# sglang-npu/DeepGEMM_Ascend

Hardware: AMD Instinct MI355X
Metric: fp8 TFLOPS + % MFMA peak, 4096^3 block-scaled GEMM; grouped-GEMM tok/s at 1/2/4/8 GPU (higher is better)
Workload: dtype bf16

## Files before the change

### deepgemm_ascend_amd/csrc/dga_launch_menu_l.hip

```cpp
#include <cstdlib>
#include "dga_fp8_menu_impl.hpp"
#include "gemm_fp8_bf16x_grouped_kernel.hpp"
namespace dga {

template <bool KTAIL, bool BNT, bool STAG, bool IDX = false>
static int launch_bf16x_grouped_one(const GemmParams &p, hipStream_t stream)
{
    typedef GemmCfg<128, 256, 2, 4, 3> Cfg;
    constexpr int kLds = Cfg::LDS_BYTES + (IDX ? 256 * 16 : 0);
    const int64_t tiles = static_cast<int64_t>(p.groups) * p.tiles_m * p.tiles_n;
    const unsigned grid = static_cast<unsigned>(std::min<int64_t>(tiles, device_cus()));
    return launch_kernel<gemm_fp8_bf16x_grouped_kernel<KTAIL, BNT, STAG, IDX>>(grid, Cfg::NT, kLds, stream, p);
}

int launch_bf16x_grouped(const GemmParams &p, hipStream_t stream)
{
    if (p.tail_sub || p.m_indices || p.launch_tiles > 0 || p.splitk > 1 || p.kb_n < 2) return DGA_E_TILING;
    const bool nt = p.b_nt != 0;
#ifdef DGA_BXG_KNOBS
    if (const char *e = std::getenv("DGA_BXG_KNOB"); e && (std::atoi(e) & 2)) {
        if (p.k % 128) return nt ? launch_bf16x_grouped_one<true, true, false>(p, stream) : launch_bf16x_grouped_one<true, false, false>(p, stream);
        return nt ? launch_bf16x_grouped_one<false, true, false>(p, stream) : launch_bf16x_grouped_one<false, false, false>(p, stream);
    }
#endif
    if (p.row_index) {
        if (p.k % 128) return nt ? launch_bf16x_grouped_one<true, true, true, true>(p, stream) : launch_bf16x_grouped_one<true, false, true, true>(p, stream);
        return nt ? launch_bf16x_grouped_one<false, true, true, true>(p, stream) : launch_bf16x_grouped_one<false, false, true, true>(p, stream);
    }
    if (p.k % 128) return nt ? launch_bf16x_grouped_one<true, true, true>(p, stream) : launch_bf16x_grouped_one<true, false, true>(p, stream);
    return nt ? launch_bf16x_grouped_one<false, true, true>(p, stream) : launch_bf16x_grouped_one<false, false, true>(p, stream);
}
}
```

### deepgemm_ascend_amd/csrc/gemm_fp8_bf16x_grouped_kernel.hpp

```cpp
#pragma once
#include "gemm_fp8_kernel.hpp"

namespace dga {

template <bool KTAIL, bool BNT, bool STAGGER = true, bool INDEXED = false>
__global__ void __launch_bounds__(512) __attribute__((amdgpu_waves_per_eu(2, 2)))
gemm_fp8_bf16x_grouped_kernel(const GemmParams p)
{
    typedef GemmCfg<128, 256, 2, 4, 3> Cfg;
    constexpr int BM = Cfg::kBM, BN = Cfg::kBN, WN = Cfg::kWN, TM = Cfg::TM, TN = Cfg::TN, DNT = Cfg::DNT;
    constexpr int NL = Cfg::LOADS_PER_STAGE, LAGT = 2, RING = 4, NT = Cfg::NT;
    static_assert(Cfg::NT == 512 && DNT == 512 && TM == 4 && TN == 4 && Cfg::SC_ITERS == 1 && Cfg::STAGES == 3, "the grouped schedule");
    typedef __bf16 v8bf __attribute__((ext_vector_type(8)));
    extern __shared__ __attribute__((aligned(16))) uint8_t smem[];

    const int tid = threadIdx.x, lane = tid & 63;
    const int wave = __builtin_amdgcn_readfirstlane(tid >> 6);
    const int wm = wave / WN, wn = wave % WN;
    const int li = lane & 15, kg = lane >> 4;
    const int KB = p.kb_n;

    const int tiles_per_group = p.tiles_m * p.tiles_n;
    const int total = p.groups * tiles_per_group;
    int first = 0, count = total, step = gridDim.x, slot = blockIdx.x;
    if (p.xcd_remap) {
        const int xcd = blockIdx.x & 7, q = total >> 3, r = total & 7;
        first = xcd < r ? xcd * (q + 1) : r * (q + 1) + (xcd - r) * q;
        count = q + (xcd < r ? 1 : 0);
        step = ((int)gridDim.x - xcd + 7) >> 3;
        slot = blockIdx.x >> 3;
    }
    struct Tile { int g, M, m0, n0; };
    typedef const __attribute__((address_space(4))) int32_t *const_i32_ptr;
    const const_i32_ptr masked_m_c = (const_i32_ptr)p.masked_m;
    auto seek = [&](int &local, Tile &t) -> bool {
        for (; local < count; local += step) {
            const int tile = first + local;
            const int g = tile / tiles_per_group;
            const int t_in = tile - g * tiles_per_group;
            const int gm = p.raster_group;
            const int per = gm * p.tiles_n;
            const int band = t_in / per;
            const int row0 = band * gm;
            const int rows = min(p.tiles_m - row0, gm);
            const int loc = t_in - band * per;
            const int tm = row0 + loc % rows, tn = loc / rows;
            const int M = p.masked_m ? min(masked_m_c[g], p.m) : p.m;
            const int m0 = tm * BM;
            if (m0 >= M) continue;
            t.g = g; t.M = M; t.m0 = m0; t.n0 = tn * BN;
            return true;
        }
        return false;
    };

    const uint32_t lds0 = (uint32_t)(uintptr_t)(lptr_t)smem;
    constexpr uint32_t kOutOfRange = 0x80000000u;
    const int a_col = ((tid & 7) ^ swz_a(tid >> 3)) * 16;
    const int b_col = ((tid & 7) ^ swz_b(tid >> 3)) * 16;
    v4i a_rsrc, b_rsrc;
    uint32_t a_voff[Cfg::A_ITERS], b_voff[Cfg::B_ITERS];
    const float *sc_src;
    int kbf = 0;
    bool fill_valid = true;
    constexpr bool indexed = INDEXED;
    static_assert(Cfg::A_ITERS == 2, "partner slot: two A offsets and the scale pointer");
    uint32_t *const pslot = reinterpret_cast<uint32_t *>(smem + Cfg::LDS_BYTES) + (tid & (DNT / 2 - 1)) * 4;
    auto a_off_of = [&](const Tile &t, int it, int td) -> uint32_t {
        const int row = (it * DNT + td) >> 3;
        if (row >= t.M - t.m0) return kOutOfRange;
        const uint32_t r = indexed ? (uint32_t)p.row_index[(int64_t)t.g * p.m + t.m0 + row] : (uint32_t)row;
        return r * (uint32_t)p.lda + a_col;
    };
    auto b_off_of = [&](const Tile &t, int it, int td) -> uint32_t {
        const int row = (it * DNT + td) >> 3;
        return (uint32_t)min(row, p.n - 1 - t.n0) * (uint32_t)p.ldb + b_col;
    };
    auto sc_of = [&](const Tile &t, int td) -> const float * {
        const float *SFA = p.sfa + (int64_t)t.g * p.sfa_gs, *SFB = p.sfb + (int64_t)t.g * p.sfb_gs;
        if (td >= BM) return SFB + (int64_t)min(t.n0 / 128 + min(td - BM, 7), p.nb_n - 1) * p.kb_n;
        const int mr = min(t.m0 + td, t.M - 1);
        return SFA + (indexed ? p.row_index[(int64_t)t.g * p.m + mr] : (int64_t)mr) * p.sfa_ld;
    };
    Tile T{}, F{};
    auto set_fill = [&](const Tile &t) {
        a_rsrc = indexed ? make_rsrc(p.a, p.a_bytes)
                         : make_rsrc(p.a + (int64_t)t.g * p.a_gs + (int64_t)t.m0 * p.lda, (int64_t)(t.M - t.m0) * p.lda);
        b_rsrc = make_rsrc(p.b + (int64_t)t.g * p.b_gs + (int64_t)t.n0 * p.ldb, (int64_t)(p.n - t.n0) * p.ldb);
#pragma unroll
        for (int it = 0; it < Cfg::A_ITERS; ++it) a_voff[it] = a_off_of(t, it, tid);
#pragma unroll
        for (int it = 0; it < Cfg::B_ITERS; ++it) b_voff[it] = b_off_of(t, it, tid);
        sc_src = sc_of(t, tid);
        if constexpr (INDEXED) {
            if (wm == 1) {
                const uint64_t ps = (uint64_t)(uintptr_t)sc_of(t, tid - DNT / 2);
                *reinterpret_cast<v4i *>(pslot) = v4i{(int)a_off_of(t, 0, tid - DNT / 2), (int)a_off_of(t, 1, tid - DNT / 2), (int)(uint32_t)ps, (int)(uint32_t)(ps >> 32)};
            }
        }
    };
    auto refill = [&](int idx, int stage, auto sc) {
        constexpr int S = decltype(sc)::value;
        const int w = wave - 4 * S, td = tid - S * (DNT / 2);
        const uint32_t sa = lds0 + stage * Cfg::STAGE_BYTES + w * 1024;
        const int k0 = kbf * 128;
        if (idx < Cfg::A_ITERS) {
            uint32_t voff = fill_valid ? (S ? (INDEXED ? pslot[idx] : a_off_of(F, idx, td)) : a_voff[idx]) : kOutOfRange;
            if constexpr (KTAIL) voff = (k0 + a_col < p.k) ? voff : kOutOfRange;
            dma16(voff, a_rsrc, (uint32_t)k0, sa + idx * DNT * 16);
        } else if (idx < Cfg::A_ITERS + Cfg::B_ITERS) {
            const int it = idx - Cfg::A_ITERS;
            uint32_t voff = fill_valid ? (S ? b_off_of(F, it, td) : b_voff[it]) : kOutOfRange;
            if constexpr (KTAIL) voff = (k0 + b_col < p.k) ? voff : kOutOfRange;
            if constexpr (BNT) dma16_nt(voff, b_rsrc, (uint32_t)k0, sa + Cfg::A_BYTES + it * DNT * 16);
            else dma16(voff, b_rsrc, (uint32_t)k0, sa + Cfg::A_BYTES + it * DNT * 16);
        } else {
            const float *src = S ? (INDEXED ? reinterpret_cast<const float *>((uintptr_t)*reinterpret_cast<const uint64_t *>(pslot + 2)) : sc_of(F, td)) : sc_src;
            dma4(src + (fill_valid ? kbf : KB - 1), lds0 + stage * Cfg::STAGE_BYTES + Cfg::A_BYTES + Cfg::B_BYTES + w * 256);
        }
    };
    constexpr std::integral_constant<int, 0> kOwn{};
    constexpr std::integral_constant<int, 1> kPartner{};

    const int a_row = wm * (BM / Cfg::kWM) + li;
    const int a_off0 = a_row * 128 + ((kg ^ swz_a(a_row)) * 16);
    const int a_off1 = a_row * 128 + (((kg + 4) ^ swz_a(a_row)) * 16);
    const int b_row = wn * (BN / WN) + 8 * (li >> 2) + (li & 3);
    const int b_off0 = Cfg::A_BYTES + b_row * 128 + ((kg ^ swz_b(b_row)) * 16);
    const int b_off1 = Cfg::A_BYTES + b_row * 128 + (((kg + 4) ^ swz_b(b_row)) * 16);
    const int sa_off = Cfg::A_BYTES + Cfg::B_BYTES + (wm * (BM / Cfg::kWM) + li) * 4;
    const int sb_off = Cfg::A_BYTES + Cfg::B_BYTES + (BM + (wn * (BN / WN)) / 128) * 4;

    v4f acc[TM][TN];
    v4f part[RING];
    v4i afx[TM][4], bfx[2][4];
    v4i braw[2], araw[2][2];
    float s_cur[TM], s_old[TM];

    auto wait_all_but = [&](auto base, int extra) {
        constexpr int B = decltype(base)::value;
        if (extra >= 8) wait_vmcnt<B + 8>();
        else if (extra >= 6) wait_vmcnt<B + 6>();
        else if (extra >= 4) wait_vmcnt<B + 4>();
        else if (extra >= 2) wait_vmcnt<B + 2>();
        else wait_vmcnt<B>();
    };
    auto wait_landed = [&](int younger, int extra) {
        if (younger >= 2 * NL) wait_all_but(std::integral_constant<int, 2 * NL>{}, extra);
        else if (younger >= NL) wait_all_but(std::integral_constant<int, NL>{}, extra);
        else wait_all_but(std::integral_constant<int, 0>{}, extra);
    };

    int local = slot;
    if (!seek(local, T)) return;
    F = T;
    set_fill(F);
#pragma unroll
    for (int d = 0; d < 2; ++d) {
#pragma unroll
        for (int idx = 0; idx < NL; ++idx) refill(idx, d, kOwn);
        ++kbf;
    }
    int cur = 0;
    DGA_STAMP_DECL
    DGA_STAMP_CLOCK(6, 7);
    DGA_STAMP_START();
    int stores_pending = 0;
    int younger = NL;

    auto advance_fill = [&]() {
        if (kbf == KB) {
            local += step;
            fill_valid = seek(local, F);
            if (fill_valid) set_fill(F);
            kbf = 0;
        }
    };

    auto run_tile = [&](auto Lc, auto lonec, auto stagc) __attribute__((always_inline)) {
        constexpr int L = decltype(Lc)::value;
        constexpr bool lone = decltype(lonec)::value;
        constexpr bool STAG = decltype(stagc)::value;
        constexpr int G = 4 * (L > 0 ? L : 1);
        constexpr int TILES = (L > 0 ? L : 1) * TN;
        constexpr int SP = L > 0 ? L : 1;
        constexpr int HALF = 2 * TILES;
        static_assert(1 + (NL - 1) * SP < HALF, "the refill fits half a block");
        static_assert(!(STAG && (lone || L == 0)), "a staggered wave multiplies and issues its own pieces");
        if constexpr (L > 0) {
#pragma unroll
            for (int i = 0; i < L; ++i)
#pragma unroll
                for (int j = 0; j < TN; ++j) acc[i][j] = v4f{0.f, 0.f, 0.f, 0.f};
#pragma unroll
            for (int i = 0; i < RING; ++i) part[i] = v4f{0.f, 0.f, 0.f, 0.f};
#pragma unroll
            for (int i = 0; i < L; ++i) s_old[i] = 0.f;
        }
        auto head = [&](const uint8_t *sc) __attribute__((always_inline)) {
            araw[0][0] = *(const v4i *)(sc + a_off0);
            araw[0][1] = *(const v4i *)(sc + a_off1);
            braw[0] = *(const v4i *)(sc + b_off0);
            braw[1] = *(const v4i *)(sc + b_off1);
            if constexpr (L > 1) {
                araw[1][0] = *(const v4i *)(sc + a_off0 + 2048);
                araw[1][1] = *(const v4i *)(sc + a_off1 + 2048);
            }
            const float sfb0 = *(const float *)(sc + sb_off);
            float sa[L > 0 ? L : 1];
#pragma unroll
            for (int i = 0; i < L; ++i) sa[i] = *(const float *)(sc + sa_off + i * 64);
            __builtin_amdgcn_sched_barrier(0);
#pragma unroll
            for (int c = 0; c < 8; ++c) bx_convert(braw, bfx[0], c);
            braw[0] = *(const v4i *)(sc + b_off0 + b_frag_off(1));
#pragma unroll
            for (int c = 8; c < 16; ++c) bx_convert(braw, bfx[0], c);
            braw[1] = *(const v4i *)(sc + b_off1 + b_frag_off(1));
#pragma unroll
            for (int c = 0; c < 16; ++c) bx_convert(araw[0], afx[0], c);
            if constexpr (L > 2) {
                araw[0][0] = *(const v4i *)(sc + a_off0 + 2 * 2048);
                araw[0][1] = *(const v4i *)(sc + a_off1 + 2 * 2048);
            }
#pragma unroll
            for (int i = 0; i < L; ++i) s_cur[i] = sa[i] * sfb0;
            __builtin_amdgcn_sched_barrier(0);
        };
        auto gaps = [&](auto u0c, auto u1c, auto refillc, const uint8_t *sc, int fill) __attribute__((always_inline)) {
            constexpr int U0 = decltype(u0c)::value, U1 = decltype(u1c)::value;
            constexpr bool REFILL = decltype(refillc)::value;
#pragma unroll
            for (int u = U0; u < U1; ++u) {
                const int t = u >> 2, q = u & 3, nt = t / L, mt = t % L, g = u % G;
                part[t % RING] = __builtin_amdgcn_mfma_f32_16x16x32_bf16(
                    __builtin_bit_cast(v8bf, bfx[nt & 1][q]), __builtin_bit_cast(v8bf, afx[mt][q]),
                    q == 0 ? v4f{0.f, 0.f, 0.f, 0.f} : part[t % RING], 0, 0, 0);
                __builtin_amdgcn_sched_barrier(0);
                if (REFILL && u - U0 >= 1 && (u - U0 - 1) % SP == 0 && (u - U0 - 1) / SP < NL) refill((u - U0 - 1) / SP, fill, kOwn);
                if (nt == 0 && mt + 1 < L) {
#pragma unroll
                    for (int c = 0; c < 4; ++c) bx_convert(araw[(mt + 1) & 1], afx[mt + 1], 4 * q + c);
                    if (q == 3 && mt + 3 < L) {
                        araw[(mt + 1) & 1][0] = *(const v4i *)(sc + a_off0 + (mt + 3) * 2048);
                        araw[(mt + 1) & 1][1] = *(const v4i *)(sc + a_off1 + (mt + 3) * 2048);
                    }
                }
                if (nt + 1 < TN) {
#pragma unroll
                    for (int c = 16 * g / G; c < 16 * (g + 1) / G; ++c) bx_convert(braw, bfx[(nt + 1) & 1], c);
                    if (nt + 2 < TN) {
                        if (g == G / 2 - 1) braw[0] = *(const v4i *)(sc + b_off0 + b_frag_off(nt + 2));
                        if (g == G - 1) braw[1] = *(const v4i *)(sc + b_off1 + b_frag_off(nt + 2));
                    }
                }
                {
                    const int j = t >= LAGT ? t - LAGT : TILES + t - LAGT, jn = j / L, jm = j % L;
                    const float sv = t >= LAGT ? s_cur[jm] : s_old[jm];
                    acc[jm][jn][q] = __builtin_fmaf(part[j % RING][q], sv, acc[jm][jn][q]);
                }
                __builtin_amdgcn_sched_barrier(0);
            }
        };
        constexpr std::integral_constant<int, 0> kU0{};
        constexpr std::integral_constant<int, HALF> kUh{};
        constexpr std::integral_constant<int, 4 * TILES> kU1{};
        auto end_of_block = [&]() {
#pragma unroll
            for (int i = 0; i < L; ++i) s_old[i] = s_cur[i];
        };
        auto top = [&](int kb) __attribute__((always_inline)) -> int {
            DGA_STAMP(0);
            wait_landed(younger, kb < 2 ? stores_pending : 0);
            DGA_STAMP(1);
            __builtin_amdgcn_s_barrier();
            asm volatile("" ::: "memory");
            DGA_STAMP(2);
            advance_fill();
            return cur >= 1 ? cur - 1 : 2;
        };
        auto next_block = [&]() {
            ++kbf;
            cur = cur == 2 ? 0 : cur + 1;
        };
        if constexpr (STAG) {
            {
                const int fill = top(0);
                younger = NL;
#pragma unroll
                for (int idx = 0; idx < NL; ++idx) refill(idx, fill, kOwn);
                const uint8_t *sc = smem + cur * Cfg::STAGE_BYTES;
                head(sc);
                gaps(kU0, kUh, std::false_type{}, sc, fill);
                next_block();
            }
            for (int kb = 1; kb < KB; ++kb) {
                const int fill = top(kb);
                const uint8_t *sc = smem + cur * Cfg::STAGE_BYTES;
                gaps(kUh, kU1, std::true_type{}, sc, fill);
                end_of_block();
                head(sc);
                DGA_STAMP(3);
                gaps(kU0, kUh, std::false_type{}, sc, fill);
                DGA_STAMP(4);
                next_block();
            }
            gaps(kUh, kU1, std::false_type{}, smem, 0);
            end_of_block();
        } else {
            for (int kb = 0; kb < KB; ++kb) {
                const int fill = top(kb);
                if constexpr (L == 0) {
#pragma unroll
                    for (int idx = 0; idx < NL; ++idx) {
                        if (lone) refill(idx, fill, kPartner);
                        refill(idx, fill, kOwn);
                    }
                    younger = lone ? 2 * NL : NL;
                } else {
                    younger = lone ? 0 : NL;
                    const uint8_t *sc = smem + cur * Cfg::STAGE_BYTES;
                    head(sc);
                    DGA_STAMP(3);
                    if constexpr (lone) gaps(kU0, kU1, std::false_type{}, sc, fill);
                    else gaps(kU0, kU1, std::true_type{}, sc, fill);
                    end_of_block();
                    DGA_STAMP(4);
                }
                next_block();
            }
        }
        stores_pending = 0;
        if constexpr (L > 0) {
#pragma unroll
            for (int t = 0; t < LAGT; ++t) {
                const int j = TILES + t - LAGT, jn = j / L, jm = j % L;
#pragma unroll
                for (int q = 0; q < 4; ++q) acc[jm][jn][q] = __builtin_fmaf(part[j % RING][q], s_old[jm], acc[jm][jn][q]);
            }
            uint16_t *C = p.out + (int64_t)T.g * p.c_gs;
            const int m_row = T.m0 + wm * (BM / Cfg::kWM) + li;
            const int n_base = T.n0 + wn * (BN / WN) + 8 * kg;
            const bool vec_ok = ((p.ldc & 7) == 0) && ((((uintptr_t)C) & 15) == 0);
            if (vec_ok && T.n0 + BN <= p.n) stores_pending = 2 * L;
#pragma unroll
            for (int mt = 0; mt < L; ++mt) {
                const int m = m_row + mt * 16;
                if (m >= T.M) continue;
                uint16_t *crow = C + (indexed ? p.row_index[(int64_t)T.g * p.m + m] : (int64_t)m) * p.ldc;
#pragma unroll
                for (int j = 0; j < TN / 2; ++j) {
                    const int n = n_base + 32 * j;
                    const v4f lo = acc[mt][2 * j], hi = acc[mt][2 * j + 1];
                    const v2bf h0 = __builtin_convertvector(v2f{lo.x, lo.y}, v2bf);
                    const v2bf h1 = __builtin_convertvector(v2f{lo.z, lo.w}, v2bf);
                    const v2bf h2 = __builtin_convertvector(v2f{hi.x, hi.y}, v2bf);
                    const v2bf h3 = __builtin_convertvector(v2f{hi.z, hi.w}, v2bf);
                    const v4i pk = v4i{__builtin_bit_cast(int, h0), __builtin_bit_cast(int, h1),
                                       __builtin_bit_cast(int, h2), __builtin_bit_cast(int, h3)};
                    if (vec_ok && n + 8 <= p.n) {
                        if (p.out_nt == 1) asm volatile("global_store_dwordx4 %0, %1, off nt" :: "v"(crow + n), "v"(pk) : "memory");
                        else if (p.out_nt == 2) asm volatile("global_store_dwordx4 %0, %1, off sc0 sc1" :: "v"(crow + n), "v"(pk) : "memory");
                        else if (p.out_nt == 3) asm volatile("global_store_dwordx4 %0, %1, off sc0 sc1 nt" :: "v"(crow + n), "v"(pk) : "memory");
                        else asm volatile("global_store_dwordx4 %0, %1, off" :: "v"(crow + n), "v"(pk) : "memory");
                    } else {
                        const uint16_t *e = (const uint16_t *)&pk;
#pragma unroll
                        for (int q = 0; q < 8; ++q)
                            if (n + q < p.n) crow[n + q] = e[q];
                    }
                }
            }
        }
    };

    for (;;) {
        const int rows = T.M - T.m0 - wm * (BM / Cfg::kWM);
        const int L = rows <= 0 ? 0 : (rows >= 64 ? 4 : (rows + 15) >> 4);
        const bool lone = T.M - T.m0 <= BM / Cfg::kWM;
        constexpr std::true_type yes{};
        constexpr std::false_type no{};
        if (lone) {
            if (L == 0) run_tile(std::integral_constant<int, 0>{}, yes, no);
            else if (L == 1) run_tile(std::integral_constant<int, 1>{}, yes, no);
            else if (L == 2) run_tile(std::integral_constant<int, 2>{}, yes, no);
            else if (L == 3) run_tile(std::integral_constant<int, 3>{}, yes, no);
            else run_tile(std::integral_constant<int, 4>{}, yes, no);
        } else if (wm == 0) {
            run_tile(std::integral_constant<int, 4>{}, no, no);
        } else {
            constexpr std::integral_constant<bool, STAGGER> st{};
            if (L == 1) run_tile(std::integral_constant<int, 1>{}, no, st);
            else if (L == 2) run_tile(std::integral_constant<int, 2>{}, no, st);
            else if (L == 3) run_tile(std::integral_constant<int, 3>{}, no, st);
            else run_tile(std::integral_constant<int, 4>{}, no, st);
        }
        if (!fill_valid) break;
        T = F;
    }
    DGA_STAMP(5);
    DGA_STAMP_CLOCK(6, 7);
    DGA_STAMP_FLUSH();
    wait_vmcnt<0>();
}

}
```

Baseline: 1201.

## Prefetch grouped-GEMM row indices into an LDS ring one tile ahead

For the indexed (row-gather) grouped kernel, the row_index entries of the next tile are DMA'd into a three-slot LDS ring while the current tile computes. A-offset, scale-pointer and epilogue store-row lookups then read from LDS instead of issuing dependent global loads. The aim is to take the global-memory latency of the index gather off the tile-switch and epilogue critical path. In exchange it adds LDS footprint, slot-rotation bookkeeping, and a correctness risk if the DMA has not completed before the slot is read or if the slot bookkeeping is wrong at the end of the tile sequence.

```diff
diff --git a/deepgemm_ascend_amd/csrc/dga_launch_menu_l.hip b/deepgemm_ascend_amd/csrc/dga_launch_menu_l.hip
--- a/deepgemm_ascend_amd/csrc/dga_launch_menu_l.hip
+++ b/deepgemm_ascend_amd/csrc/dga_launch_menu_l.hip
@@ -7,7 +7,8 @@
 static int launch_bf16x_grouped_one(const GemmParams &p, hipStream_t stream)
 {
     typedef GemmCfg<128, 256, 2, 4, 3> Cfg;
-    constexpr int kLds = Cfg::LDS_BYTES + (IDX ? 256 * 16 : 0);
+    constexpr int kLds = Cfg::LDS_BYTES + (IDX ? 256 * 16 + 3 * 128 * 8 : 0);
+    static_assert(kLds <= 160 * 1024 && Cfg::LDS_BYTES % 16 == 0, "LDS of one CU; 16-byte carve offsets");
     const int64_t tiles = static_cast<int64_t>(p.groups) * p.tiles_m * p.tiles_n;
     const unsigned grid = static_cast<unsigned>(std::min<int64_t>(tiles, device_cus()));
     return launch_kernel<gemm_fp8_bf16x_grouped_kernel<KTAIL, BNT, STAG, IDX>>(grid, Cfg::NT, kLds, stream, p);
diff --git a/deepgemm_ascend_amd/csrc/gemm_fp8_bf16x_grouped_kernel.hpp b/deepgemm_ascend_amd/csrc/gemm_fp8_bf16x_grouped_kernel.hpp
--- a/deepgemm_ascend_amd/csrc/gemm_fp8_bf16x_grouped_kernel.hpp
+++ b/deepgemm_ascend_amd/csrc/gemm_fp8_bf16x_grouped_kernel.hpp
@@ -33,8 +33,8 @@
     struct Tile { int g, M, m0, n0; };
     typedef const __attribute__((address_space(4))) int32_t *const_i32_ptr;
     const const_i32_ptr masked_m_c = (const_i32_ptr)p.masked_m;
-    auto seek = [&](int &local, Tile &t) -> bool {
-        for (; local < count; local += step) {
+    auto tile_at = [&](int local, Tile &t) -> bool {
+        {
             const int tile = first + local;
             const int g = tile / tiles_per_group;
             const int t_in = tile - g * tiles_per_group;
@@ -47,10 +47,14 @@
             const int tm = row0 + loc % rows, tn = loc / rows;
             const int M = p.masked_m ? min(masked_m_c[g], p.m) : p.m;
             const int m0 = tm * BM;
-            if (m0 >= M) continue;
+            if (m0 >= M) return false;
             t.g = g; t.M = M; t.m0 = m0; t.n0 = tn * BN;
             return true;
         }
+    };
+    auto seek = [&](int &local, Tile &t) -> bool {
+        for (; local < count; local += step)
+            if (tile_at(local, t)) return true;
         return false;
     };
 
@@ -66,10 +70,17 @@
     constexpr bool indexed = INDEXED;
     static_assert(Cfg::A_ITERS == 2, "partner slot: two A offsets and the scale pointer");
     uint32_t *const pslot = reinterpret_cast<uint32_t *>(smem + Cfg::LDS_BYTES) + (tid & (DNT / 2 - 1)) * 4;
+    constexpr int kIdxBase = Cfg::LDS_BYTES + (DNT / 2) * 16, kIdxSlotBytes = BM * 8;
+    static_assert(kIdxBase % 16 == 0 && kIdxSlotBytes % 16 == 0 && BM * 2 == DNT / 2, "index slots: one dword per thread of four waves");
+    auto index_at = [&](int s, int row) -> int64_t {
+        asm volatile("" : "+v"(row));
+        return *reinterpret_cast<const int64_t *>(smem + kIdxBase + s * kIdxSlotBytes + row * 8);
+    };
+    int fslot = 0;
     auto a_off_of = [&](const Tile &t, int it, int td) -> uint32_t {
         const int row = (it * DNT + td) >> 3;
         if (row >= t.M - t.m0) return kOutOfRange;
-        const uint32_t r = indexed ? (uint32_t)p.row_index[(int64_t)t.g * p.m + t.m0 + row] : (uint32_t)row;
+        const uint32_t r = indexed ? (uint32_t)index_at(fslot, row) : (uint32_t)row;
         return r * (uint32_t)p.lda + a_col;
     };
     auto b_off_of = [&](const Tile &t, int it, int td) -> uint32_t {
@@ -80,7 +91,7 @@
         const float *SFA = p.sfa + (int64_t)t.g * p.sfa_gs, *SFB = p.sfb + (int64_t)t.g * p.sfb_gs;
         if (td >= BM) return SFB + (int64_t)min(t.n0 / 128 + min(td - BM, 7), p.nb_n - 1) * p.kb_n;
         const int mr = min(t.m0 + td, t.M - 1);
-        return SFA + (indexed ? p.row_index[(int64_t)t.g * p.m + mr] : (int64_t)mr) * p.sfa_ld;
+        return SFA + (indexed ? index_at(fslot, mr - t.m0) : (int64_t)mr) * p.sfa_ld;
     };
     Tile T{}, F{};
     auto set_fill = [&](const Tile &t) {
@@ -151,9 +162,24 @@
         else wait_all_but(std::integral_constant<int, 0>{}, extra);
     };
 
+    auto fetch_index = [&](const Tile &t, int s) {
+        if (wm == 1) {
+            const int td = tid - DNT / 2;
+            const int64_t *e = p.row_index + (int64_t)t.g * p.m + t.m0 + min(td >> 1, p.m - 1 - t.m0);
+            dma4(reinterpret_cast<const uint32_t *>(e) + (td & 1), lds0 + kIdxBase + s * kIdxSlotBytes + (wave - 4) * 256);
+        }
+    };
     int local = slot;
     if (!seek(local, T)) return;
     F = T;
+    if constexpr (INDEXED) {
+        if (tid < BM) reinterpret_cast<int64_t *>(smem + kIdxBase)[tid] = p.row_index[(int64_t)T.g * p.m + T.m0 + min(tid, p.m - 1 - T.m0)];
+        Tile N;
+        local += step;
+        const bool next_valid = seek(local, N);
+        __syncthreads();
+        if (next_valid) fetch_index(N, 1);
+    }
     set_fill(F);
 #pragma unroll
     for (int d = 0; d < 2; ++d) {
@@ -170,9 +196,20 @@
 
     auto advance_fill = [&]() {
         if (kbf == KB) {
-            local += step;
-            fill_valid = seek(local, F);
-            if (fill_valid) set_fill(F);
+            if constexpr (INDEXED) {
+                fill_valid = local < count && tile_at(local, F);
+                if (fill_valid) {
+                    fslot = fslot == 2 ? 0 : fslot + 1;
+                    Tile N;
+                    local += step;
+                    if (seek(local, N)) fetch_index(N, fslot == 2 ? 0 : fslot + 1);
+                    set_fill(F);
+                }
+            } else {
+                local += step;
+                fill_valid = seek(local, F);
+                if (fill_valid) set_fill(F);
+            }
             kbf = 0;
         }
     };
@@ -341,13 +378,14 @@
             uint16_t *C = p.out + (int64_t)T.g * p.c_gs;
             const int m_row = T.m0 + wm * (BM / Cfg::kWM) + li;
             const int n_base = T.n0 + wn * (BN / WN) + 8 * kg;
+            const int tslot = !fill_valid ? fslot : (fslot == 0 ? 2 : fslot - 1);
             const bool vec_ok = ((p.ldc & 7) == 0) && ((((uintptr_t)C) & 15) == 0);
             if (vec_ok && T.n0 + BN <= p.n) stores_pending = 2 * L;
 #pragma unroll
             for (int mt = 0; mt < L; ++mt) {
                 const int m = m_row + mt * 16;
                 if (m >= T.M) continue;
-                uint16_t *crow = C + (indexed ? p.row_index[(int64_t)T.g * p.m + m] : (int64_t)m) * p.ldc;
+                uint16_t *crow = C + (indexed ? index_at(tslot, m - T.m0) : (int64_t)m) * p.ldc;
 #pragma unroll
                 for (int j = 0; j < TN / 2; ++j) {
                     const int n = n_base + 32 * j;
```

Measured after the change: 1188. -1.1%, worse.
